# duyhominhnguyen/conan-fgw

Hardware: AMD Instinct MI355X
Metric: molecules/s (K=5 conformers) (higher is better)
Workload: dtype f32

## Files before the change

conan-fgw_amd/csrc/fgw_common.h:

```cpp
#pragma once
#include <type_traits>
#include "common.h"

#ifdef CONAN_FGW_PROFILE
static __device__ long long g_fgw_prof[32];
#define FGW_PROF_ACCESSOR(name)                                                          \
    extern "C" int name(long long *out, int reset) {                                     \
        if (out && hipMemcpyFromSymbol(out, HIP_SYMBOL(g_fgw_prof), sizeof(long long) * 32) != hipSuccess) return -2; \
        if (reset) { long long z[32] = {0}; if (hipMemcpyToSymbol(HIP_SYMBOL(g_fgw_prof), z, sizeof(z)) != hipSuccess) return -2; } \
        return 0;                                                                        \
    }
static __device__ long long g_fgw_trace[2 + 6 * 8192];
#define FGW_PROF_TRACE_ACCESSOR(name)                                                    \
    extern "C" int name(long long *out, int reset) {                                     \
        if (out && hipMemcpyFromSymbol(out, HIP_SYMBOL(g_fgw_trace), sizeof(long long) * (2 + 6 * 8192)) != hipSuccess) return -2; \
        if (reset) { long long z[2] = {0, 0}; if (hipMemcpyToSymbol(HIP_SYMBOL(g_fgw_trace), z, sizeof(z)) != hipSuccess) return -2; } \
        return 0;                                                                        \
    }
#define FGW_PROF_TRACE(tag)                                                              \
    do {                                                                                 \
        if (threadIdx.x == 0) {                                                          \
            const unsigned long long i_ = atomicAdd(reinterpret_cast<unsigned long long *>(&g_fgw_trace[0]), 1ull); \
            if (i_ < 8192) {                                                             \
                long long *r_ = &g_fgw_trace[2 + 6 * i_];                                \
// ... 100 lines not shown
    const double n = rint(t);
    const float f = (float)(t - n);
    const float e = __builtin_amdgcn_exp2f(f);
    return ldexp((double)e, (int)n);
}

__device__ __forceinline__ double exp_fast(double x) {
    const double xc = fmin(fmax(x, -700.0), 700.0);
    const double t = xc * 1.4426950408889634074;
    const double sh = t + 6755399441055744.0;
    const int n = __double2loint(sh);
    const double f = t - (sh - 6755399441055744.0);
    const double e = (double)__builtin_amdgcn_exp2f((float)f);
    const double scale = __hiloint2double((n + 1023) << 20, 0);
    const double r = e * scale;
    return x > -700.0 ? (x < 700.0 ? r : __builtin_inf()) : 0.0;
}

__device__ __forceinline__ double rcp_pos(double s) {
    double r = __builtin_amdgcn_rcp(s);
    r = fma(fma(-s, r, 1.0), r, r);
    r = fma(fma(-s, r, 1.0), r, r);
    return r;
}

__device__ __forceinline__ double log_acc(double s) {
    const double y0 = (double)(__builtin_amdgcn_logf((float)s) * 0.693147180559945309f);
    const double r = s * exp_acc(-y0) - 1.0;
    return y0 + (r - 0.5 * r * r);
}

__device__ __forceinline__ double wave_sum_d(double v) {
#pragma unroll
    for (int o = 32; o > 0; o >>= 1) v += __shfl_xor(v, o, 64);
    return v;
}
__device__ __forceinline__ double wave_max_d(double v) {
#pragma unroll
    for (int o = 32; o > 0; o >>= 1) { double w = __shfl_xor(v, o, 64); v = w > v ? w : v; }
    return v;
}

template <int NW = FGW_WAVES>
__device__ __forceinline__ double block_sum_d(double v, double *red) {
    v = wave_sum_d(v);
    __syncthreads();
    if ((threadIdx.x & 63) == 0) red[threadIdx.x >> 6] = v;
    __syncthreads();
    double s = 0.0;
#pragma unroll
    for (int w = 0; w < NW; ++w) s += red[w];
    return s;
}


typedef double f64x4 __attribute__((ext_vector_type(4)));

__device__ __forceinline__ double exp_lse(double x) {
    const float f = (float)x;
    return (double)__builtin_amdgcn_exp2f(f * 1.44269504088896340736f);
}

template <int NW = FGW_WAVES, class FX, class FW, class FS>
__device__ __forceinline__ void mm_f64_pad(int M, int Nn, int Kd, FX X, FW W, FS st) {
    const int lane = threadIdx.x & 63, wave = __builtin_amdgcn_readfirstlane((int)(threadIdx.x >> 6));
    const int Mq = (M + 15) >> 4, Nq = (Nn + 15) >> 4;
    const int li = lane & 15, lk = lane >> 4;
    for (int t = wave; t < Mq * Nq; t += NW) {
        const int i0 = (t / Nq) << 4, j0 = (t % Nq) << 4;
        const int ia = i0 + li, jb = j0 + li;
        const bool ra = ia < M, cb = jb < Nn;
        const int ic = ra ? ia : M - 1, jc = cb ? jb : Nn - 1;
        f64x4 acc = {0.0, 0.0, 0.0, 0.0};
        int k0 = 0;
        for (; k0 + 16 <= Kd; k0 += 16) {
            double a[4], b[4];
#pragma unroll
            for (int u = 0; u < 4; ++u) { a[u] = X(ic, k0 + 4 * u + lk); b[u] = W(k0 + 4 * u + lk, jc); }
#pragma unroll
            for (int u = 0; u < 4; ++u) acc = __builtin_amdgcn_mfma_f64_16x16x4f64(ra ? a[u] : 0.0, cb ? b[u] : 0.0, acc, 0, 0, 0);
        }
        if (k0 < Kd) {
            double a[4], b[4];
#pragma unroll
            for (int u = 0; u < 4; ++u) {
                const int k = k0 + 4 * u + lk, kc = k < Kd ? k : Kd - 1;
                a[u] = X(ic, kc); b[u] = W(kc, jc);
            }
#pragma unroll
            for (int u = 0; u < 4; ++u) {
                const bool kin = k0 + 4 * u + lk < Kd;
                if (k0 + 4 * u < Kd)
                    acc = __builtin_amdgcn_mfma_f64_16x16x4f64((ra && kin) ? a[u] : 0.0, (cb && kin) ? b[u] : 0.0, acc, 0, 0, 0);
            }
        }
#pragma unroll
        for (int q = 0; q < 4; ++q) {
            const int i = i0 + lk + 4 * q;
            if (i < M && cb) st(i, jb, acc[q]);
        }
    }
}

template <int NW, bool WT, typename TX, typename TW, class FS>
__device__ __forceinline__ void mm_f64_glb(int M, int Nn, int Kd, const TX *__restrict__ X, int pX, const TW *__restrict__ W, int pW, FS st,
                                           const int tid = threadIdx.x) {
    const int lane = tid & 63, wave = __builtin_amdgcn_readfirstlane(tid >> 6);
    const int Mq = (M + 15) >> 4, Nq = (Nn + 15) >> 4;
    const int li = lane & 15, lk = lane >> 4;
    for (int t = wave; t < Mq * Nq; t += NW) {
        const int i0 = (t / Nq) << 4, j0 = (t % Nq) << 4;
        const int ia = i0 + li, jb = j0 + li;
        const bool ra = ia < M, cb = jb < Nn;
        const TX *xr = X + (size_t)(ra ? ia : M - 1) * pX;
        const int jc = cb ? jb : Nn - 1;
        f64x4 acc = {0.0, 0.0, 0.0, 0.0}, acc2 = {0.0, 0.0, 0.0, 0.0};
        for (int k0 = 0; k0 < Kd; k0 += 16) {
            const int kb = k0 + 4 * lk;
            double a[4], b[4];
            if (k0 + 16 <= Kd) {
#pragma unroll
                for (int u = 0; u < 4; ++u) a[u] = (double)xr[kb + u];
                if (WT) {
                    const TW *wr = W + (size_t)jc * pW + kb;
#pragma unroll
                    for (int u = 0; u < 4; ++u) b[u] = (double)wr[u];
                } else {
#pragma unroll
                    for (int u = 0; u < 4; ++u) b[u] = (double)W[(size_t)(kb + u) * pW + jc];
                }
            } else {
#pragma unroll
                for (int u = 0; u < 4; ++u) {
                    const int k = kb + u, kc = k < Kd ? k : Kd - 1;
                    const double av = (double)xr[kc], bv = (double)(WT ? W[(size_t)jc * pW + kc] : W[(size_t)kc * pW + jc]);
                    a[u] = k < Kd ? av : 0.0; b[u] = k < Kd ? bv : 0.0;
                }
            }
            acc = __builtin_amdgcn_mfma_f64_16x16x4f64(ra ? a[0] : 0.0, cb ? b[0] : 0.0, acc, 0, 0, 0);
            acc2 = __builtin_amdgcn_mfma_f64_16x16x4f64(ra ? a[1] : 0.0, cb ? b[1] : 0.0, acc2, 0, 0, 0);
            acc = __builtin_amdgcn_mfma_f64_16x16x4f64(ra ? a[2] : 0.0, cb ? b[2] : 0.0, acc, 0, 0, 0);
            acc2 = __builtin_amdgcn_mfma_f64_16x16x4f64(ra ? a[3] : 0.0, cb ? b[3] : 0.0, acc2, 0, 0, 0);
        }
#pragma unroll
        for (int q = 0; q < 4; ++q) {
            const int i = i0 + lk + 4 * q;
            if (i < M && cb) st(i, jb, acc[q] + acc2[q]);
        }
    }
}

template <int NT>
__device__ __forceinline__ void fgw_order_by_size(const FgwAdj &adj, int B, int K, int tid) {
    static_assert(NT >= 256, "one thread per size bin");
    __shared__ unsigned char nsz[4096];
    __shared__ int hist[256], base[256];
    if (B > 4096) return;
    for (int t = tid; t < 256; t += NT) hist[t] = 0;
    __syncthreads();
    for (int m = tid; m < B; m += NT) {
        const int n = min(max(adj.gptr[m * K + 1] - adj.gptr[m * K], 0), 255);
        nsz[m] = (unsigned char)n;
        atomicAdd(&hist[n], 1);
    }
    __syncthreads();
    if (tid == 0) {
        int run = 0;
        for (int v = 255; v >= 0; --v) { base[v] = run; run += hist[v]; }
    }
    __syncthreads();
    if (tid < 256 && hist[tid] > 0) {
        int pos = base[tid];
        for (int m = 0; m < B; ++m)
            if (nsz[m] == (unsigned char)tid) adj.order[pos++] = m;
    }
}

#ifndef CONAN_FGW_KT
#define CONAN_FGW_KT 2
#endif
template <int NW, bool WT, typename TX, typename TW, class FS, int KT = CONAN_FGW_KT>
__device__ __forceinline__ void mm_f64_glb22(int M, int Nn, int Kd, const TX *__restrict__ X, int pX, const TW *__restrict__ W, int pW, FS st,
                                             const int tid = threadIdx.x) {
    const int lane = tid & 63, wave = __builtin_amdgcn_readfirstlane(tid >> 6);
    const int Mq = (M + 15) >> 4, Nq = (Nn + 15) >> 4;
    const int li = lane & 15, lk = lane >> 4;
    const int Mb = Mq >> 1, Nb = Nq >> 1;
    const int nblk = Mb * Nb, nblk_used = (nblk / NW) * NW;
    auto load_a = [&](const TX *xr, int kb, int k0, double (&a)[KT]) {
        if (k0 + 4 * KT <= Kd) {
#pragma unroll
            for (int u = 0; u < KT; ++u) a[u] = (double)xr[kb + u];
        } else {
#pragma unroll
            for (int u = 0; u < KT; ++u) { const int k = kb + u; const double v = (double)xr[k < Kd ? k : Kd - 1]; a[u] = k < Kd ? v : 0.0; }
        }
    };
    auto load_b = [&](int jc, int kb, int k0, double (&b)[KT]) {
        if (k0 + 4 * KT <= Kd) {
#pragma unroll
            for (int u = 0; u < KT; ++u) b[u] = (double)(WT ? W[(size_t)jc * pW + kb + u] : W[(size_t)(kb + u) * pW + jc]);
        } else {
#pragma unroll
            for (int u = 0; u < KT; ++u) {
                const int k = kb + u, kc = k < Kd ? k : Kd - 1;
                const double v = (double)(WT ? W[(size_t)jc * pW + kc] : W[(size_t)kc * pW + jc]);
                b[u] = k < Kd ? v : 0.0;
            }
        }
    };
    auto store_tile = [&](int i0, int j0, const f64x4 &r) {
        const int jb = j0 + li;
        if (jb < Nn) {
#pragma unroll
            for (int q = 0; q < 4; ++q) { const int i = i0 + lk + 4 * q; if (i < M) st(i, jb, r[q]); }
        }
    };
    for (int t = wave; t < nblk_used; t += NW) {
        const int i0 = (t / Nb) << 5, j0 = (t % Nb) << 5;
        const TX *x0 = X + (size_t)min(i0 + li, M - 1) * pX, *x1 = X + (size_t)min(i0 + 16 + li, M - 1) * pX;
        const int jc0 = min(j0 + li, Nn - 1), jc1 = min(j0 + 16 + li, Nn - 1);
        f64x4 c00 = {0.0, 0.0, 0.0, 0.0}, c01 = c00, c10 = c00, c11 = c00;
        for (int k0 = 0; k0 < Kd; k0 += 4 * KT) {
            const int kb = k0 + KT * lk;
            double a0[KT], a1[KT], b0[KT], b1[KT];
            load_a(x0, kb, k0, a0); load_a(x1, kb, k0, a1); load_b(jc0, kb, k0, b0); load_b(jc1, kb, k0, b1);
#pragma unroll
            for (int u = 0; u < KT; ++u) {
                c00 = __builtin_amdgcn_mfma_f64_16x16x4f64(a0[u], b0[u], c00, 0, 0, 0);
                c01 = __builtin_amdgcn_mfma_f64_16x16x4f64(a0[u], b1[u], c01, 0, 0, 0);
                c10 = __builtin_amdgcn_mfma_f64_16x16x4f64(a1[u], b0[u], c10, 0, 0, 0);
                c11 = __builtin_amdgcn_mfma_f64_16x16x4f64(a1[u], b1[u], c11, 0, 0, 0);
            }
        }
        store_tile(i0, j0, c00); store_tile(i0, j0 + 16, c01); store_tile(i0 + 16, j0, c10); store_tile(i0 + 16, j0 + 16, c11);
    }
    const int rest_blk = nblk - nblk_used;
    const int n_single = rest_blk * 4 + (Mq * Nq - 4 * nblk);
    for (int t = wave; t < n_single; t += NW) {
        int ti, tj;
        if (t < rest_blk * 4) { const int bq = nblk_used + (t >> 2); ti = 2 * (bq / Nb) + ((t >> 1) & 1); tj = 2 * (bq % Nb) + (t & 1); }
        else {
            int q = t - rest_blk * 4;
            const int ncol = (Nq & 1) ? Mq : 0;
            if (q < ncol) { ti = q; tj = Nq - 1; }
            else { q -= ncol; ti = Mq - 1; tj = q; }
        }
        const int i0 = ti << 4, j0 = tj << 4;
        const TX *xr = X + (size_t)min(i0 + li, M - 1) * pX;
        const int jc = min(j0 + li, Nn - 1);
        f64x4 acc = {0.0, 0.0, 0.0, 0.0}, acc2 = {0.0, 0.0, 0.0, 0.0};
        for (int k0 = 0; k0 < Kd; k0 += 4 * KT) {
            const int kb = k0 + KT * lk;
            double a[KT], bq[KT];
            load_a(xr, kb, k0, a); load_b(jc, kb, k0, bq);
#pragma unroll
            for (int u = 0; u < KT; ++u) {
                if (u & 1) acc2 = __builtin_amdgcn_mfma_f64_16x16x4f64(a[u], bq[u], acc2, 0, 0, 0);
                else acc = __builtin_amdgcn_mfma_f64_16x16x4f64(a[u], bq[u], acc, 0, 0, 0);
            }
        }
        store_tile(i0, j0, acc + acc2);
    }
}

typedef int fgw_i32x4 __attribute__((ext_vector_type(4)));
__device__ __forceinline__ void fgw_digit_planes4(const double (&v)[4], double scale, unsigned (&pl)[4]) {
    unsigned r[4];
#pragma unroll
    for (int u = 0; u < 4; ++u) r[u] = ((unsigned)__double2int_rn(v[u] * scale) + 0x00808080u) ^ 0x00808080u;
    const unsigned t0 = __builtin_amdgcn_perm(r[1], r[0], 0x05010400u), t1 = __builtin_amdgcn_perm(r[1], r[0], 0x07030602u);
    const unsigned t2 = __builtin_amdgcn_perm(r[3], r[2], 0x05010400u), t3 = __builtin_amdgcn_perm(r[3], r[2], 0x07030602u);
    pl[0] = __builtin_amdgcn_perm(t2, t0, 0x05040100u); pl[1] = __builtin_amdgcn_perm(t2, t0, 0x07060302u);
    pl[2] = __builtin_amdgcn_perm(t3, t1, 0x05040100u); pl[3] = __builtin_amdgcn_perm(t3, t1, 0x07060302u);
}
template <int NT>
__device__ __forceinline__ void fgw_digits_from_f64(int M, int Kd, const double *__restrict__ X, int pX, int xexp, uint4 *__restrict__ D, const int tid = threadIdx.x) {
    const int KB = ((Kd + 31) >> 5) << 2;
    const double scale = __longlong_as_double((long long)(1023 + 31 - xexp) << 52);
    constexpr int R = 2;
    for (int base = 0; base < M * KB; base += R * NT) {
        double v[R][8];
#pragma unroll
        for (int q = 0; q < R; ++q) {
            const int idx = base + q * NT + tid;
            const int ic = idx < M * KB ? idx : M * KB - 1;
            const int i = ic / KB, kb = ic - i * KB;
            const double *xr = X + (size_t)i * pX;
#pragma unroll
            for (int u = 0; u < 8; ++u) { const int k = 8 * kb + u; v[q][u] = xr[k < Kd ? k : Kd - 1]; }
        }
#pragma unroll
        for (int q = 0; q < R; ++q) {
            const int idx = base + q * NT + tid;
            if (idx >= M * KB) continue;
            const int kb = idx % KB;
            double v0[4], v1[4];
#pragma unroll
            for (int u = 0; u < 4; ++u) { v0[u] = 8 * kb + u < Kd ? v[q][u] : 0.0; v1[u] = 8 * kb + 4 + u < Kd ? v[q][4 + u] : 0.0; }
            unsigned lo[4], hi[4];
            fgw_digit_planes4(v0, scale, lo); fgw_digit_planes4(v1, scale, hi);
            D[2 * idx] = make_uint4(lo[0], hi[0], lo[1], hi[1]);
            D[2 * idx + 1] = make_uint4(lo[2], hi[2], lo[3], hi[3]);
        }
    }
}
__device__ __forceinline__ long fgw_bytes8(const unsigned char *__restrict__ w, int kb, int Kd) {
    unsigned lo = 0, hi = 0;
#pragma unroll
    for (int u = 0; u < 4; ++u) {
        const int k0 = kb + u, k1 = kb + 4 + u;
        lo |= (unsigned)w[k0 < Kd ? k0 : Kd - 1] << (8 * u);
        hi |= (unsigned)w[k1 < Kd ? k1 : Kd - 1] << (8 * u);
    }
    return (long)(((unsigned long long)hi << 32) | lo);
}
template <int NW, class FS>
__device__ __forceinline__ void mm_adj_i8(int M, int Nn, int Kd, const uint4 *__restrict__ D, const unsigned char *__restrict__ Wb, int pW, int xexp, FS st,
                                          const int tid = threadIdx.x) {
    const int lane = tid & 63, wave = __builtin_amdgcn_readfirstlane(tid >> 6);
    const int li = lane & 15, lg = lane >> 4;
    const int Mq = (M + 15) >> 4, Nh = (Nn + 31) >> 5, KB = ((Kd + 31) >> 5) << 2;
    const double unscale = __longlong_as_double((long long)(1023 + xexp - 31) << 52);
    for (int t = wave; t < Mq * Nh; t += NW) {
        const int i0 = (t / Nh) << 4, j0 = (t % Nh) << 5;
        const uint4 *dr = D + (size_t)min(i0 + li, M - 1) * KB * 2;
        const unsigned char *w0 = Wb + (size_t)min(j0 + li, Nn - 1) * pW, *w1 = Wb + (size_t)min(j0 + 16 + li, Nn - 1) * pW;
// ... 559 lines not shown
```

conan-fgw_amd/csrc/fgw_small.hip:

```cpp
#include "fgw_common.h"

#ifdef CONAN_FGW_PROFILE
FGW_PROF_ACCESSOR(conan_debug_fgw_prof)
FGW_PROF_TRACE_ACCESSOR(conan_debug_fgw_trace)
#endif

namespace {

constexpr int SK_SCRATCH_DOUBLES = 3 * 256 + 2 * 64;

template <int R, bool KL, bool SECOND = false>
__global__ void __launch_bounds__(FGW_THREADS, (SECOND || R > 9) ? 1 : 3) k_fgw_coupling_small(
    const float *__restrict__ Ys, const float *__restrict__ Cs, const float *__restrict__ ps, const float *__restrict__ pb,
    FgwDims D, conan_fgw_params prm, int outer, int y_zero, const double *__restrict__ Cw, const double *__restrict__ Yw,
    const int *__restrict__ active, float *__restrict__ Tw, int *__restrict__ info, fgw_part_t *__restrict__ Ypart,
    fgw_part_t *__restrict__ Cpart, const double *__restrict__ zvec, const double *__restrict__ yvec, const int *__restrict__ only, FgwAdj adj) {
    extern __shared__ __attribute__((aligned(16))) char smem[];
    auto solve = [&](const int cid) {
    const int b = cid / D.K, s = cid % D.K;
    if (!fgw_active(active, D.B, b, outer)) return;
    const int N = D.N, P = D.P, d = D.d;
    const int NN = N * N, NP = N * P;
    const int tid = threadIdx.x, lane = tid & 63, w = __builtin_amdgcn_readfirstlane(tid >> 6);
    const bool lane_ok = lane < N;
// ... 663 lines not shown
            if (!have_colp) {
                double pc = 0.0;
                if (ii == 0) {
                    gvP[permL] = lq_ok ? (lq == nbq ? (double)m_pad : 1.0) : 0.0;
                }
                pc = dotR(kA, gw);
                *bufCw = pc;
                __syncthreads();
                colp = ((bufC[lq] + bufC[64 + lq]) + bufC[128 + lq]) + bufC[192 + lq];
            }
            have_colp = false;
            if (__any(lq_ok && !(colp > 1e-150 && colp < 1e150))) { bail = true; break; }
            f = lq_ok ? qj * rcp_pos(colp) : 0.0;
            fvP[permL] = f;
            *bufRw = dotR(kB, fw);
            __syncthreads();
            const double rs = ((bufR[lq] + bufR[64 + lq]) + bufR[128 + lq]) + bufR[192 + lq];
            if (__any(lq_ok && !(rs > 1e-150 && rs < 1e150))) { bail = true; break; }
            g = lq_ok ? pi_l * rcp_pos(rs) : 0.0;
            gvP[permL] = g;
            if (ii % 10 == 0) {
                *bufCw = dotR(kA, gw);
                __syncthreads();
                colp = ((bufC[lq] + bufC[64 + lq]) + bufC[128 + lq]) + bufC[192 + lq];
                have_colp = true;
                double df = lq_ok ? f * colp - qj : 0.0;
                df = df * df;
                if (lq == nbq) df /= (double)m_pad;
                df = wave_sum_d(df);
                if (sqrt(df) < fc.stop_thr) { ++ii; break; }
            }
        }
        if (bail) break;
        sk_total += ii;
        FGW_PROF(6);
        double e2 = 0.0;
        {
            float *trow = Tl + wq * P + lq;
#pragma unroll
            for (int r = 0; r < R; ++r) {
                const bool ok = lq_ok && wq + 4 * r < N;
                float *tp = ok ? trow + 4 * r * P : t_dummy;
                const float tn = (float)((gw[r] * kA[r]) * f);
                double df = ok ? (double)tn - (double)*tp : 0.0;
                df *= df;
                if (nbq >= 0) {
                    const double im = 1.0 / (double)m_pad;
                    df *= (lq == nbq ? im : 1.0) * (wq + 4 * r == nbq ? im : 1.0);
                }
                e2 += df;
                *tp = tn;
            }
        }
        if (cpt % 10 == 0) err = sqrt(block_sum_d(e2, red));
        else __syncthreads();
        ++cpt;
        FGW_PROF(7);
    }
    if (bail) {
        if (tid == 0) { redo[cid] = 1; atomicOr(&info[b * 4 + 3], 1); }
        return;
    }
    __syncthreads();
    {
        int te = tid;
        asm volatile("" : "+v"(te));
        int i = te / N, j = te - i * N;
        const int dq = FGW_THREADS / N, dr = FGW_THREADS - dq * N;
        if (m_pad) {
            const float im = (float)(1.0 / mult);
            for (int t = te; t < NN; t += FGW_THREADS) {
                Tg[t] = Tl[min(i, nb) * P + min(j, nb)] * ((i >= nb ? im : 1.0f) * (j >= nb ? im : 1.0f));
                j += dr; i += dq;
                if (j >= N) { j -= N; ++i; }
            }
        } else {
            for (int t = te; t < NN; t += FGW_THREADS) {
                Tg[t] = Tl[i * P + j];
                j += dr; i += dq;
                if (j >= N) { j -= N; ++i; }
            }
        }
    }
    if (tid == 0) { atomicAdd(&info[b * 4 + 1], cpt); atomicAdd(&info[b * 4 + 2], sk_total); redo[cid] = 0; if (m_pad) atomicOr(&info[b * 4 + 3], 2); }
    FGW_PROF(8);

    if (!prm.fixed_features && Ypart) {
        fgw_part_t *Yp = Ypart + ((size_t)b * D.K + s) * N * d;
        if (yz_lds) {
            const int Nd = N * d;
            for (int t0 = tid; t0 < Nd; t0 += 4 * FGW_THREADS) {
                float zv[4];
#pragma unroll
                for (int u = 0; u < 4; ++u) { const int t = t0 + u * FGW_THREADS; zv[u] = Z[t < Nd ? t : Nd - 1]; }
#pragma unroll
                for (int u = 0; u < 4; ++u) { const int t = t0 + u * FGW_THREADS; if (t < Nd) Zl[t] = zv[u]; }
            }
            __syncthreads();
            mm_lds2<FGW_WAVES, 1, 0, false, false>(N, d, N, Tl, P, Zl, d, [] {}, [&](int i, int c, double v) { Yp[(size_t)i * d + c] = (fgw_part_t)v; });
        } else {
            mm_f64(N, d, N, [&](int i, int k) { return (double)Tl[i * P + k]; }, [&](int k, int c) { return (double)Z[(size_t)k * d + c]; },
                   [&](int i, int c, double v) { Yp[(size_t)i * d + c] = (fgw_part_t)v; });
        }
    }
    FGW_PROF(9);
    if (!prm.fixed_structure) {
        fgw_part_t *Cp = Cpart + ((size_t)b * D.K + s) * NN;
        if (complete) {
            {
                const int lc = lane < Nx ? lane : Nx - 1;
                const float *tr = Tl + lc * P + w;
                double p0 = 0.0, p1 = 0.0;
#pragma unroll
                for (int r = 0; r < R; ++r) {
                    const int q = w + 4 * r;
                    if (q < n_real) { if (r & 1) p1 += (double)tr[4 * r]; else p0 += (double)tr[4 * r]; }
                }
                if (lane < Nx) rsum[w * N + lane] = p0 + p1;
            }
            __syncthreads();
            mm_lds2<FGW_WAVES, 1, 0, true, false>(Nx, Nx, n_real, Tl, P, Tl, P, [] {}, [&](int i, int j, double v) {
                const double ti = ((rsum[i] + rsum[N + i]) + rsum[2 * N + i]) + rsum[3 * N + i];
                const double tj = ((rsum[j] + rsum[N + j]) + rsum[2 * N + j]) + rsum[3 * N + j];
                if (m_pad) Bl[i * P + j] = ti * tj - v;
                else Cp[i * N + j] = (fgw_part_t)(ti * tj - v);
            });
        } else {
            mm_lds2<FGW_WAVES, 1, 0, false, false>(Nx, Nx, Nx, Tl, P, C2l, P, [] {}, [&](int i, int j, double v) { AKl[i * P + j] = v; });
            __syncthreads();
            mm_lds2<FGW_WAVES, 1, 0, true, false>(Nx, Nx, Nx, AKl, P, Tl, P, [] {}, [&](int i, int j, double v) {
                if (m_pad) Bl[i * P + j] = v;
                else Cp[i * N + j] = (fgw_part_t)v;
            });
        }
        if (m_pad) {
            __syncthreads();
            const double im = 1.0 / mult;
            int i = tid / N, j = tid - i * N;
            const int dq = FGW_THREADS / N, dr = FGW_THREADS - dq * N;
            for (int t = tid; t < NN; t += FGW_THREADS) {
                Cp[t] = (fgw_part_t)(Bl[min(i, nb) * P + min(j, nb)] * ((i >= nb ? im : 1.0) * (j >= nb ? im : 1.0)));
                j += dr; i += dq;
                if (j >= N) { j -= N; ++i; }
            }
        }
    }
    FGW_PROF(10);
    FGW_PROF_FLUSH;
    FGW_PROF_TRACE(Nx | (cpt << 8) | (sk_total << 20));
}

template <int NT>
__device__ __forceinline__ void molecule_vectors(const double *__restrict__ Y, const double *__restrict__ C, const float *__restrict__ p, int N,
                                                 int d, bool kl, double *__restrict__ out, int which = 2) {
    constexpr int LPI = NT / 64;
    const int i = (int)threadIdx.x / LPI, sub = (int)threadIdx.x % LPI;
    double y2 = 0.0, r1 = 0.0;
    if (i < N) {
        if (which != 1)
            for (int c = sub; c < d; c += LPI) { const double v = Y[(size_t)i * d + c]; y2 += v * v; }
        if (which != 0)
            for (int k = sub; k < N; k += LPI) {
                const double c1 = C[i * N + k], pk = p ? (double)p[k] : 1.0 / (double)N;
                r1 += (kl ? c1 * log(c1 + 1e-15) - c1 : c1 * c1) * pk;
            }
    }
#pragma unroll
    for (int o = 1; o < LPI; o <<= 1) { y2 += __shfl_xor(y2, o, 64); r1 += __shfl_xor(r1, o, 64); }
    if (i < N && sub == 0) { if (which != 1) out[i] = y2; if (which != 0) out[N + i] = r1; }
}

__global__ void __launch_bounds__(256) k_fgw_small_vectors(const float *__restrict__ Ys, const float *__restrict__ Cs, const float *__restrict__ ps,
                                                           const float *__restrict__ pb, FgwDims D, int kl, double *__restrict__ Cw,
                                                           double *__restrict__ Yw, double *__restrict__ zvec, double *__restrict__ yvec,
                                                           const float *__restrict__ init_C, const float *__restrict__ init_Y, int max_iter,
                                                           int *__restrict__ active, int *__restrict__ info, float *__restrict__ errs,
                                                           float *__restrict__ Yout, float *__restrict__ Cout, FgwAdj adj) {
    const int b = blockIdx.x / D.K, s = blockIdx.x % D.K;
    const int N = D.N, d = D.d;
    __shared__ __attribute__((aligned(16))) unsigned char cm[64 * 65 + 16];
    const int Pm = D.P;
    if (adj.rowptr) {
        for (int t = threadIdx.x; t < (64 * 65 + 16) / 4; t += 256) reinterpret_cast<unsigned *>(cm)[t] = 0u;
        __syncthreads();
        adj_scatter_lds_bytes<256>(adj, (int)blockIdx.x, N, Pm, cm, (int)threadIdx.x);
        __syncthreads();
    }
    if (s == 0) {
        const int NN = N * N, Nd = N * d;
        const float *c0 = init_C ? init_C + (size_t)b * NN : Cs + (size_t)b * D.K * NN;
        for (int t = threadIdx.x; t < NN; t += 256) {
            const float cv = (!init_C && adj.rowptr) ? (float)cm[(t / N) * Pm + (t % N)] : c0[t];
            Cw[(size_t)b * NN + t] = (double)cv; Cout[(size_t)b * NN + t] = cv;
        }
        for (int t = threadIdx.x; t < Nd; t += 256) {
            const float y = init_Y ? init_Y[(size_t)b * Nd + t] : 0.f;
            Yw[(size_t)b * Nd + t] = (double)y; Yout[(size_t)b * Nd + t] = y;
        }
        if (threadIdx.x == 0) { fgw_active_init(active, D.B, b); info[b * 4 + 0] = 0; info[b * 4 + 1] = 0; info[b * 4 + 2] = 0; info[b * 4 + 3] = 0; }
        for (int t = threadIdx.x; t < 2 * max_iter; t += 256) errs[(size_t)b * 2 * max_iter + t] = __builtin_nanf("");
        __syncthreads();
    }
    const float *Z = Ys + ((size_t)b * D.K + s) * N * d;
    const float *C2 = Cs + ((size_t)b * D.K + s) * N * N;
    const float *q = ps ? ps + ((size_t)b * D.K + s) * N : nullptr;
    const int j = (int)threadIdx.x >> 2, sub = (int)threadIdx.x & 3;
    double z2 = 0.0, r2 = 0.0;
    if (j < N) {
        for (int c = sub; c < d; c += 4) { const double v = (double)Z[(size_t)j * d + c]; z2 += v * v; }
        for (int k = sub; k < N; k += 4) {
            const double c2 = adj.rowptr ? (double)cm[j * Pm + k] : (double)C2[j * N + k], qk = q ? (double)q[k] : 1.0 / (double)N;
            r2 += qk * (kl ? c2 : c2 * c2);
        }
    }
    z2 += __shfl_xor(z2, 1, 64); z2 += __shfl_xor(z2, 2, 64);
    r2 += __shfl_xor(r2, 1, 64); r2 += __shfl_xor(r2, 2, 64);
    double *zo = zvec + ((size_t)b * D.K + s) * 2 * N;
    if (j < N && sub == 0) { zo[j] = z2; zo[N + j] = r2; }
    if (s == 0)
        molecule_vectors<256>(Yw + (size_t)b * N * d, Cw + (size_t)b * N * N, pb ? pb + (size_t)b * N : nullptr, N, d, kl != 0, yvec + (size_t)b * 2 * N);
    if (adj.order && blockIdx.x == gridDim.x - 1) fgw_order_by_size<256>(adj, D.B, D.K, (int)threadIdx.x);
}

constexpr int UPD_THREADS = 512;
template <bool Y_FROM_T>
__global__ void __launch_bounds__(UPD_THREADS) k_fgw_update_parts(
    const float *__restrict__ pb, const float *__restrict__ lambdas, FgwDims D, conan_fgw_params prm, int outer,
    const fgw_part_t *__restrict__ Ypart, const fgw_part_t *__restrict__ Cpart, double *__restrict__ Cw, double *__restrict__ Yw,
    int *__restrict__ active, int *__restrict__ info, float *__restrict__ errs, float *__restrict__ Yout, float *__restrict__ Cout,
    double *__restrict__ yvec, const float *__restrict__ Tw, const float *__restrict__ Ys, int chunk) {
    __shared__ double red[UPD_THREADS / 64 + 1];
    extern __shared__ __attribute__((aligned(16))) char usmem[];
    const int part = (int)blockIdx.x >= D.B ? 1 : 0;
    const int b = (int)blockIdx.x - part * D.B;
    const int N = D.N, d = D.d, K = D.K, NN = N * N, Nd = N * d;
    const int tid = threadIdx.x;
    int *flag_out = active + (outer & 1) * 2 * D.B + part * D.B + b;
    if (!fgw_active(active, D.B, b, outer)) {
        if (tid == 0) *flag_out = 0;
        return;
    }
    constexpr int U = 4;
    double e2 = 0.0;
    if (part == 0) {
        if (!prm.fixed_features) {
            double *Yb = Yw + (size_t)b * Nd;
            if constexpr (Y_FROM_T) {
                float *Tl = reinterpret_cast<float *>(usmem), *Zl = Tl + (size_t)chunk * NN;
                const int lane = tid & 63, wave = __builtin_amdgcn_readfirstlane(tid >> 6), li = lane & 15, lk = lane >> 4;
                const int Mq = (N + 15) >> 4, Nq = (d + 15) >> 4;
                constexpr int NWU = UPD_THREADS / 64, TW = 2;
                for (int t0 = 0; t0 < Mq * Nq; t0 += NWU * TW) {
                    int ti0[TW], tj0[TW], tic[TW], tjc[TW];
                    bool mine[TW];
                    f64x4 sum[TW];
#pragma unroll
                    for (int w = 0; w < TW; ++w) {
                        const int t = t0 + wave + w * NWU;
                        mine[w] = t < Mq * Nq;
                        ti0[w] = mine[w] ? (t / Nq) << 4 : 0; tj0[w] = mine[w] ? (t % Nq) << 4 : 0;
                        tic[w] = min(ti0[w] + li, N - 1); tjc[w] = min(tj0[w] + li, d - 1);
                        sum[w] = f64x4{0.0, 0.0, 0.0, 0.0};
                    }
                    for (int s0 = 0; s0 < K; s0 += chunk) {
                        const int cs = min(chunk, K - s0);
                        __syncthreads();
                        const float *tg = Tw + ((size_t)b * K + s0) * NN, *zg = Ys + ((size_t)b * K + s0) * Nd;
                        auto stage = [&](const float *__restrict__ src, float *dst, int n) {
                            constexpr int SB = 12;
                            for (int base = 0; base < n; base += SB * UPD_THREADS) {
                                float v[SB];
#pragma unroll
                                for (int u = 0; u < SB; ++u) { const int q = base + u * UPD_THREADS + tid; v[u] = src[q < n ? q : n - 1]; }
#pragma unroll
                                for (int u = 0; u < SB; ++u) { const int q = base + u * UPD_THREADS + tid; if (q < n) dst[q] = v[u]; }
                            }
                        };
                        stage(tg, Tl, cs * NN);
                        stage(zg, Zl, cs * Nd);
                        __syncthreads();
#pragma unroll
                        for (int w = 0; w < TW; ++w)
                            if (mine[w])
                                for (int q = 0; q < cs; ++q) {
                                    const double lam = lambdas ? (double)lambdas[s0 + q] : 1.0 / (double)K;
                                    const f64x4 r = mm2_tile<0, false>(Tl + (size_t)q * NN + tic[w] * N + lk, Zl + (size_t)q * Nd + lk * d + tjc[w], d, N, lk);
                                    sum[w] = sum[w] + lam * r;
                                }
                    }
#pragma unroll
                    for (int w = 0; w < TW; ++w) {
                        const int jb = tj0[w] + li;
                        if (mine[w] && jb < d) {
#pragma unroll
                            for (int qq = 0; qq < 4; ++qq) {
                                const int i = ti0[w] + lk + 4 * qq;
                                if (i < N) {
                                    const double pw = pb ? (double)pb[(size_t)b * N + i] : 1.0 / (double)N;
                                    const double yn = sum[w][qq] * (pw > 0.0 ? 1.0 / pw : 0.0);
                                    const double df = yn - Yb[i * d + jb];
                                    e2 += df * df;
                                    Yb[i * d + jb] = yn;
                                    Yout[(size_t)b * Nd + i * d + jb] = (float)yn;
                                }
                            }
                        }
                    }
                }
            } else {
                for (int t0 = tid; t0 < Nd; t0 += U * UPD_THREADS) {
                    double acc[U], old[U];
#pragma unroll
                    for (int u = 0; u < U; ++u) {
                        const int t = t0 + u * UPD_THREADS;
                        acc[u] = 0.0; old[u] = 0.0;
                        if (t < Nd) {
                            old[u] = Yb[t];
                            for (int s = 0; s < K; ++s) {
                                const double lam = lambdas ? (double)lambdas[s] : 1.0 / (double)K;
                                const int i = t / d;
                                const double pw = pb ? (double)pb[(size_t)b * N + i] : 1.0 / (double)N;
                                const double pinv = pw > 0.0 ? 1.0 / pw : 0.0;
                                acc[u] += lam * Ypart[((size_t)b * K + s) * Nd + t] * pinv;
                            }
                        }
                    }
#pragma unroll
                    for (int u = 0; u < U; ++u) {
                        const int t = t0 + u * UPD_THREADS;
                        if (t < Nd) {
                            const double df = acc[u] - old[u];
                            e2 += df * df;
                            Yb[t] = acc[u];
                            Yout[(size_t)b * Nd + t] = (float)acc[u];
                        }
                    }
                }
            }
        }
    } else if (!prm.fixed_structure) {
        double *Cb = Cw + (size_t)b * NN;
        for (int t0 = tid; t0 < NN; t0 += U * UPD_THREADS) {
            double acc[U], old[U];
#pragma unroll
            for (int u = 0; u < U; ++u) {
                const int t = t0 + u * UPD_THREADS;
                acc[u] = 0.0; old[u] = 0.0;
                if (t < NN) {
                    old[u] = Cb[t];
                    for (int s = 0; s < K; ++s) {
                        const double lam = lambdas ? (double)lambdas[s] : 1.0 / (double)K;
                        acc[u] += lam * Cpart[((size_t)b * K + s) * NN + t];
                    }
                }
            }
#pragma unroll
            for (int u = 0; u < U; ++u) {
                const int t = t0 + u * UPD_THREADS;
                if (t < NN) {
                    const int i = t / N, j = t - i * N;
                    const double pi = pb ? (double)pb[(size_t)b * N + i] : 1.0 / (double)N;
                    const double pj = pb ? (double)pb[(size_t)b * N + j] : 1.0 / (double)N;
                    const double cn = pi * pj > 0.0 ? (prm.loss_fun ? exp(acc[u] / (pi * pj)) : acc[u] / (pi * pj)) : 0.0;
                    const double df = cn - old[u];
                    e2 += df * df;
                    Cb[t] = cn;
                    Cout[(size_t)b * NN + t] = (float)cn;
                }
            }
        }
    }
    const double err = sqrt(block_sum_d<UPD_THREADS / 64>(e2, red));
    if (yvec) molecule_vectors<UPD_THREADS>(Yw + (size_t)b * Nd, Cw + (size_t)b * NN, pb ? pb + (size_t)b * N : nullptr, N, d, prm.loss_fun != 0,
                                            yvec + (size_t)b * 2 * N, part);
    if (tid == 0) {
        errs[((size_t)b * 2 + part) * prm.max_iter + outer] = (float)err;
        info[b * 4 + 0] = outer + 1;
        *flag_out = err > (double)prm.tol ? 1 : 0;
    }
}

inline size_t small_lds(int N, int d) {
    const size_t NP = (size_t)N * fgw_pitch(N);
    (void)d; return NP * 8 * 4 + (256 + 128 + 8 + (NP >= (size_t)SK_SCRATCH_DOUBLES ? 0 : SK_SCRATCH_DOUBLES)) * 8 + NP * 4 * 2;
}

}

bool conan_fgw_small_supported(int N, int d) { return N <= 64 && small_lds(N, d) <= 160 * 1024; }

void conan_fgw_small_prepare(const FgwCall &c) {
    k_fgw_small_vectors<<<c.D.B * c.D.K, 256, 0, c.s>>>(c.Ys, c.Cs, c.ps, c.p, c.D, c.prm.loss_fun, c.Cw, c.Yw, c.zvec, c.yvec, c.init_C, c.init_Y,
                                                       c.prm.max_iter, c.active, c.info, c.errs, c.Y, c.C, c.adj);
}

template <class F>
static void with_rows(int R, F &&f) {
    if (R <= 6) f(std::integral_constant<int, 6>{});
    else if (R <= 9) f(std::integral_constant<int, 9>{});
    else if (R <= 12) f(std::integral_constant<int, 12>{});
    else f(std::integral_constant<int, 16>{});
}

template <int R, typename C2T>
static void launch_fast(const FgwCall &c, int outer, int y_zero, fgw_part_t *Ypart) {
    const FgwDims &D = c.D;
    const int tpw = fast_tiles_per_wave(D.N);
    auto go = [&](auto kernel) {
        launch_lds(kernel, D.B * D.K, FGW_THREADS, fast_lds<C2T>(D.N).bytes, c.s, c.Ys, c.Cs, c.ps, c.p, D, c.prm, fast_const(c.prm, D.N), outer,
                   y_zero, c.Cw, c.Yw, c.active, c.T, c.info, Ypart, c.Cpart, c.zvec, c.yvec, c.redo, c.adj);
    };
    if constexpr (R <= 6) go(k_fgw_coupling_fast<R, 1, C2T>);
    else if constexpr (R <= 12) { if (tpw <= 1) go(k_fgw_coupling_fast<R, 1, C2T>); else go(k_fgw_coupling_fast<R, 3, C2T>); }
    else { if (tpw <= 1) go(k_fgw_coupling_fast<R, 1, C2T>); else if (tpw <= 3) go(k_fgw_coupling_fast<R, 3, C2T>); else go(k_fgw_coupling_fast<R, 4, C2T>); }
}

bool conan_fgw_fast_supported(int N, int d, int small_int) {
    if (N > 64 || N < 4) return false;
    const size_t lds = small_int ? fast_lds<unsigned char>(N).bytes : fast_lds<float>(N).bytes;
    return lds <= 160 * 1024 && d >= 1;
}

void conan_fgw_small_coupling(const FgwCall &c, int outer, int y_zero, fgw_part_t *Ypart) {
    const FgwDims &D = c.D;
    const size_t lds = small_lds(D.N, D.d);
    const int grid = D.B * D.K;
    const bool kl = c.prm.loss_fun != 0;
    with_rows((D.N + 3) / 4, [&](auto R) {
        const int *only = nullptr;
        if (!kl && conan_fgw_fast_supported(D.N, D.d, c.prm.cs_small_int)) {
            if (c.prm.cs_small_int) launch_fast<R.value, unsigned char>(c, outer, y_zero, Ypart);
            else launch_fast<R.value, float>(c, outer, y_zero, Ypart);
            only = c.redo;
        }
        auto exact = [&](auto kernel, int blocks) {
            launch_lds(kernel, blocks, FGW_THREADS, lds, c.s, c.Ys, c.Cs, c.ps, c.p, D, c.prm, outer, y_zero, c.Cw, c.Yw, c.active, c.T, c.info, Ypart,
                       c.Cpart, c.zvec, c.yvec, only, c.adj);
        };
        if (kl) exact(k_fgw_coupling_small<R.value, true, false>, grid);
        else if (only) exact(k_fgw_coupling_small<R.value, false, true>, (grid + 63) / 64);
        else exact(k_fgw_coupling_small<R.value, false, false>, grid);
    });
}

void conan_fgw_small_update(const FgwCall &c, int outer, bool y_from_t) {
    const FgwDims &D = c.D;
    const int chunk = y_from_t ? conan_fgw_update_chunk(D.K, D.N, D.d, D.B) : 0;
    if (chunk > 0)
        launch_lds(k_fgw_update_parts<true>, 2 * D.B, UPD_THREADS, (size_t)chunk * ((size_t)D.N * D.N + (size_t)D.N * D.d) * 4, c.s, c.p, c.lambdas, D,
                   c.prm, outer, nullptr, c.Cpart, c.Cw, c.Yw, c.active, c.info, c.errs, c.Y, c.C, c.yvec, c.T, c.Ys, chunk);
    else
        k_fgw_update_parts<false><<<2 * D.B, UPD_THREADS, 0, c.s>>>(c.p, c.lambdas, D, c.prm, outer, c.Ypart, c.Cpart, c.Cw, c.Yw, c.active, c.info, c.errs,
                                                                     c.Y, c.C, c.yvec, nullptr, nullptr, 0);
}

int conan_fgw_update_chunk(int K, int N, int d, int B) {
    if (N > 64) return 0;
    const size_t per = ((size_t)N * N + (size_t)N * d) * 4, budget = (2 * B <= 256 ? 144 : 72) * 1024;
    if (per > budget) return 0;
    const int c = (int)(budget / per);
    return c < K ? c : K;
}
```

Measured before the change: 118,200.

## Parallelize size ordering, fuse T/Z staging and reuse LDS results in update

Replaces the serial per-bin scan in fgw_order_by_size with a parallel prefix scan and a wavefront-level packed-byte rank, and runs it in a dedicated extra workgroup at the start of the grid instead of the last block. The update kernel now stages T and Z in one fused batched loop, issues its global loads before checking the active flag, and prefetches the old Y values and pb entries. It also writes the updated Y and C into LDS so molecule_vectors reads them from there rather than from global memory, and adds an occupancy hint to the launch bounds. The intent is to cut serial latency and global round trips, at the cost of extra LDS, more registers and loads issued for inactive molecules.

```diff
diff --git a/conan-fgw_amd/csrc/fgw_common.h b/conan-fgw_amd/csrc/fgw_common.h
--- a/conan-fgw_amd/csrc/fgw_common.h
+++ b/conan-fgw_amd/csrc/fgw_common.h
@@ -276,27 +276,72 @@
 
 template <int NT>
 __device__ __forceinline__ void fgw_order_by_size(const FgwAdj &adj, int B, int K, int tid) {
-    static_assert(NT >= 256, "one thread per size bin");
-    __shared__ unsigned char nsz[4096];
-    __shared__ int hist[256], base[256];
+    static_assert(NT >= 256 && NT % 64 == 0 && 4096 % NT == 0, "one thread per size bin, whole wavefronts, whole rounds");
+    constexpr int NWV = NT / 64, RB = 4;
+    __shared__ __attribute__((aligned(4))) unsigned char nsz[4096];
+    __shared__ int hist[256], next[256], scan[2][256];
+    __shared__ unsigned wcnt[NWV * 64];
     if (B > 4096) return;
     for (int t = tid; t < 256; t += NT) hist[t] = 0;
     __syncthreads();
-    for (int m = tid; m < B; m += NT) {
-        const int n = min(max(adj.gptr[m * K + 1] - adj.gptr[m * K], 0), 255);
-        nsz[m] = (unsigned char)n;
-        atomicAdd(&hist[n], 1);
+    for (int m0 = 0; m0 < B; m0 += RB * NT) {
+        int lo[RB], hi[RB];
+#pragma unroll
+        for (int r = 0; r < RB; ++r) {
+            const int m = min(m0 + r * NT + tid, B - 1);
+            lo[r] = adj.gptr[m * K]; hi[r] = adj.gptr[m * K + 1];
+        }
+#pragma unroll
+        for (int r = 0; r < RB; ++r) {
+            const int m = m0 + r * NT + tid;
+            if (m < B) {
+                const int n = min(max(hi[r] - lo[r], 0), 255);
+                nsz[m] = (unsigned char)n;
+                atomicAdd(&hist[n], 1);
+            }
+        }
     }
     __syncthreads();
-    if (tid == 0) {
-        int run = 0;
-        for (int v = 255; v >= 0; --v) { base[v] = run; run += hist[v]; }
-    }
+    if (tid < 256) scan[0][tid] = hist[255 - tid];
     __syncthreads();
-    if (tid < 256 && hist[tid] > 0) {
-        int pos = base[tid];
-        for (int m = 0; m < B; ++m)
-            if (nsz[m] == (unsigned char)tid) adj.order[pos++] = m;
+    int src = 0;
+    for (int off = 1; off < 256; off <<= 1) {
+        if (tid < 256) scan[src ^ 1][tid] = scan[src][tid] + (tid >= off ? scan[src][tid - off] : 0);
+        __syncthreads();
+        src ^= 1;
+    }
+    if (tid < 256) next[255 - tid] = scan[src][tid] - hist[255 - tid];
+    const int lane = tid & 63, wv = tid >> 6;
+    for (int m0 = 0; m0 < B; m0 += NT) {
+        for (int t = tid; t < NWV * 64; t += NT) wcnt[t] = 0u;
+        __syncthreads();
+        const int m = m0 + tid;
+        const bool on = m < B;
+        const int n = on ? (int)nsz[m] : 0;
+        if (on) atomicAdd(&wcnt[wv * 64 + (n >> 2)], 1u << (8 * (n & 3)));
+        int before = 0;
+        const unsigned *row = reinterpret_cast<const unsigned *>(nsz) + ((m0 + wv * 64) >> 2);
+        const unsigned n4 = (unsigned)n * 0x01010101u;
+#pragma unroll
+        for (int q = 0; q < 16; ++q) {
+            const unsigned x = row[q] ^ n4;
+            const unsigned eq = ~((((x & 0x7f7f7f7fu) + 0x7f7f7f7fu) | x) | 0x7f7f7f7fu);
+            const int k = min(max(lane - 4 * q, 0), 4);
+            before += __popc(eq & (unsigned)(0x80808080ull & ((1ull << (8 * k)) - 1ull)));
+        }
+        __syncthreads();
+        if (on) {
+            int pos = next[n] + before;
+            for (int w = 0; w < wv; ++w) pos += (int)((wcnt[w * 64 + (n >> 2)] >> (8 * (n & 3))) & 255u);
+            adj.order[pos] = m;
+        }
+        int add = 0;
+        if (tid < 256) {
+#pragma unroll
+            for (int w = 0; w < NWV; ++w) add += (int)((wcnt[w * 64 + (tid >> 2)] >> (8 * (tid & 3))) & 255u);
+        }
+        __syncthreads();
+        if (tid < 256) next[tid] += add;
     }
 }
 
diff --git a/conan-fgw_amd/csrc/fgw_small.hip b/conan-fgw_amd/csrc/fgw_small.hip
--- a/conan-fgw_amd/csrc/fgw_small.hip
+++ b/conan-fgw_amd/csrc/fgw_small.hip
@@ -839,16 +839,17 @@
 
 template <int NT>
 __device__ __forceinline__ void molecule_vectors(const double *__restrict__ Y, const double *__restrict__ C, const float *__restrict__ p, int N,
-                                                 int d, bool kl, double *__restrict__ out, int which = 2) {
+                                                 int d, bool kl, double *__restrict__ out, int which,
+                                                 int pY, int pC) {
     constexpr int LPI = NT / 64;
     const int i = (int)threadIdx.x / LPI, sub = (int)threadIdx.x % LPI;
     double y2 = 0.0, r1 = 0.0;
     if (i < N) {
         if (which != 1)
-            for (int c = sub; c < d; c += LPI) { const double v = Y[(size_t)i * d + c]; y2 += v * v; }
+            for (int c = sub; c < d; c += LPI) { const double v = Y[(size_t)i * pY + c]; y2 += v * v; }
         if (which != 0)
             for (int k = sub; k < N; k += LPI) {
-                const double c1 = C[i * N + k], pk = p ? (double)p[k] : 1.0 / (double)N;
+                const double c1 = C[i * pC + k], pk = p ? (double)p[k] : 1.0 / (double)N;
                 r1 += (kl ? c1 * log(c1 + 1e-15) - c1 : c1 * c1) * pk;
             }
     }
@@ -863,14 +864,16 @@
                                                            const float *__restrict__ init_C, const float *__restrict__ init_Y, int max_iter,
                                                            int *__restrict__ active, int *__restrict__ info, float *__restrict__ errs,
                                                            float *__restrict__ Yout, float *__restrict__ Cout, FgwAdj adj) {
-    const int b = blockIdx.x / D.K, s = blockIdx.x % D.K;
+    const int wg = (int)blockIdx.x - (adj.order ? 1 : 0);
+    if (wg < 0) { fgw_order_by_size<256>(adj, D.B, D.K, (int)threadIdx.x); return; }
+    const int b = wg / D.K, s = wg % D.K;
     const int N = D.N, d = D.d;
     __shared__ __attribute__((aligned(16))) unsigned char cm[64 * 65 + 16];
     const int Pm = D.P;
     if (adj.rowptr) {
         for (int t = threadIdx.x; t < (64 * 65 + 16) / 4; t += 256) reinterpret_cast<unsigned *>(cm)[t] = 0u;
         __syncthreads();
-        adj_scatter_lds_bytes<256>(adj, (int)blockIdx.x, N, Pm, cm, (int)threadIdx.x);
+        adj_scatter_lds_bytes<256>(adj, wg, N, Pm, cm, (int)threadIdx.x);
         __syncthreads();
     }
     if (s == 0) {
@@ -905,17 +908,16 @@
     double *zo = zvec + ((size_t)b * D.K + s) * 2 * N;
     if (j < N && sub == 0) { zo[j] = z2; zo[N + j] = r2; }
     if (s == 0)
-        molecule_vectors<256>(Yw + (size_t)b * N * d, Cw + (size_t)b * N * N, pb ? pb + (size_t)b * N : nullptr, N, d, kl != 0, yvec + (size_t)b * 2 * N);
-    if (adj.order && blockIdx.x == gridDim.x - 1) fgw_order_by_size<256>(adj, D.B, D.K, (int)threadIdx.x);
+        molecule_vectors<256>(Yw + (size_t)b * N * d, Cw + (size_t)b * N * N, pb ? pb + (size_t)b * N : nullptr, N, d, kl != 0, yvec + (size_t)b * 2 * N, 2, d, N);
 }
 
 constexpr int UPD_THREADS = 512;
 template <bool Y_FROM_T>
-__global__ void __launch_bounds__(UPD_THREADS) k_fgw_update_parts(
+__global__ void __launch_bounds__(UPD_THREADS, 4) k_fgw_update_parts(
     const float *__restrict__ pb, const float *__restrict__ lambdas, FgwDims D, conan_fgw_params prm, int outer,
     const fgw_part_t *__restrict__ Ypart, const fgw_part_t *__restrict__ Cpart, double *__restrict__ Cw, double *__restrict__ Yw,
     int *__restrict__ active, int *__restrict__ info, float *__restrict__ errs, float *__restrict__ Yout, float *__restrict__ Cout,
-    double *__restrict__ yvec, const float *__restrict__ Tw, const float *__restrict__ Ys, int chunk) {
+    double *__restrict__ yvec, const float *__restrict__ Tw, const float *__restrict__ Ys, int chunk, int y_lds) {
     __shared__ double red[UPD_THREADS / 64 + 1];
     extern __shared__ __attribute__((aligned(16))) char usmem[];
     const int part = (int)blockIdx.x >= D.B ? 1 : 0;
@@ -923,10 +925,14 @@
     const int N = D.N, d = D.d, K = D.K, NN = N * N, Nd = N * d;
     const int tid = threadIdx.x;
     int *flag_out = active + (outer & 1) * 2 * D.B + part * D.B + b;
-    if (!fgw_active(active, D.B, b, outer)) {
+    const bool act = fgw_active(active, D.B, b, outer);
+    const bool late = Y_FROM_T && (part == 0 ? !prm.fixed_features : !prm.fixed_structure);
+    if (!late && !act) {
         if (tid == 0) *flag_out = 0;
         return;
     }
+    double *const Xl = reinterpret_cast<double *>(usmem);
+    const int dP = d | 1, nP = N | 1;
     constexpr int U = 4;
     double e2 = 0.0;
     if (part == 0) {
@@ -949,23 +955,42 @@
                         tic[w] = min(ti0[w] + li, N - 1); tjc[w] = min(tj0[w] + li, d - 1);
                         sum[w] = f64x4{0.0, 0.0, 0.0, 0.0};
                     }
+                    double yold[TW][4];
                     for (int s0 = 0; s0 < K; s0 += chunk) {
                         const int cs = min(chunk, K - s0);
+                        if (t0 | s0) __syncthreads();
+                        const float *tg = Tw + ((size_t)b * K + s0) * NN, *zg = Ys + ((size_t)b * K + s0) * Nd;
+                        {
+                            constexpr int ST = 11, SZ = 21;
+                            const int nT = cs * NN, nZ = cs * Nd;
+                            for (int bt = 0, bz = 0; bt < nT || bz < nZ; bt += ST * UPD_THREADS, bz += SZ * UPD_THREADS) {
+                                float vt[ST], vz[SZ];
+#pragma unroll
+                                for (int u = 0; u < ST; ++u) vt[u] = tg[min(bt + u * UPD_THREADS + tid, nT - 1)];
+#pragma unroll
+                                for (int u = 0; u < SZ; ++u) vz[u] = zg[min(bz + u * UPD_THREADS + tid, nZ - 1)];
+                                if (late && !(t0 | s0 | bt) && !act) {
+                                    if (tid == 0) *flag_out = 0;
+                                    return;
+                                }
+#pragma unroll
+                                for (int u = 0; u < ST; ++u) { const int q = bt + u * UPD_THREADS + tid; if (q < nT) Tl[q] = vt[u]; }
+#pragma unroll
+                                for (int u = 0; u < SZ; ++u) { const int q = bz + u * UPD_THREADS + tid; if (q < nZ) Zl[q] = vz[u]; }
+                            }
+                        }
                         __syncthreads();
-                        const float *tg = Tw + ((size_t)b * K + s0) * NN, *zg = Ys + ((size_t)b * K + s0) * Nd;
-                        auto stage = [&](const float *__restrict__ src, float *dst, int n) {
-                            constexpr int SB = 12;
-                            for (int base = 0; base < n; base += SB * UPD_THREADS) {
-                                float v[SB];
-#pragma unroll
-                                for (int u = 0; u < SB; ++u) { const int q = base + u * UPD_THREADS + tid; v[u] = src[q < n ? q : n - 1]; }
-#pragma unroll
-                                for (int u = 0; u < SB; ++u) { const int q = base + u * UPD_THREADS + tid; if (q < n) dst[q] = v[u]; }
-                            }
-                        };
-                        stage(tg, Tl, cs * NN);
-                        stage(zg, Zl, cs * Nd);
-                        __syncthreads();
+                        if (s0 + chunk >= K) {
+                            int lkq = lk;
+                            asm volatile("" : "+v"(lkq));
+#pragma unroll
+                            for (int w = 0; w < TW; ++w)
+#pragma unroll
+                                for (int qq = 0; qq < 4; ++qq) {
+                                    const int ic = min(ti0[w] + lkq + 4 * qq, N - 1);
+                                    yold[w][qq] = Yb[ic * d + tjc[w]];
+                                }
+                        }
 #pragma unroll
                         for (int w = 0; w < TW; ++w)
                             if (mine[w])
@@ -975,6 +1000,10 @@
                                     sum[w] = sum[w] + lam * r;
                                 }
                     }
+                    if (y_lds) __syncthreads();
+                    int Nu = N;
+                    asm volatile("" : "+s"(Nu));
+                    const double pw_uniform = 1.0 / (double)Nu;
 #pragma unroll
                     for (int w = 0; w < TW; ++w) {
                         const int jb = tj0[w] + li;
@@ -983,12 +1012,13 @@
                             for (int qq = 0; qq < 4; ++qq) {
                                 const int i = ti0[w] + lk + 4 * qq;
                                 if (i < N) {
-                                    const double pw = pb ? (double)pb[(size_t)b * N + i] : 1.0 / (double)N;
+                                    const double pw = pb ? (double)pb[(size_t)b * N + i] : pw_uniform;
                                     const double yn = sum[w][qq] * (pw > 0.0 ? 1.0 / pw : 0.0);
-                                    const double df = yn - Yb[i * d + jb];
+                                    const double df = yn - yold[w][qq];
                                     e2 += df * df;
                                     Yb[i * d + jb] = yn;
                                     Yout[(size_t)b * Nd + i * d + jb] = (float)yn;
+                                    if (y_lds) Xl[i * dP + jb] = yn;
                                 }
                             }
                         }
@@ -1027,39 +1057,52 @@
         }
     } else if (!prm.fixed_structure) {
         double *Cb = Cw + (size_t)b * NN;
-        for (int t0 = tid; t0 < NN; t0 += U * UPD_THREADS) {
+        for (int r0 = 0; r0 < NN; r0 += U * UPD_THREADS) {
+            const int t0 = r0 + tid;
             double acc[U], old[U];
+            float pfi[U], pfj[U];
 #pragma unroll
             for (int u = 0; u < U; ++u) {
                 const int t = t0 + u * UPD_THREADS;
-                acc[u] = 0.0; old[u] = 0.0;
+                acc[u] = 0.0; old[u] = 0.0; pfi[u] = 0.f; pfj[u] = 0.f;
                 if (t < NN) {
                     old[u] = Cb[t];
+                    if (pb) { const int i = t / N; pfi[u] = pb[(size_t)b * N + i]; pfj[u] = pb[(size_t)b * N + (t - i * N)]; }
                     for (int s = 0; s < K; ++s) {
                         const double lam = lambdas ? (double)lambdas[s] : 1.0 / (double)K;
                         acc[u] += lam * Cpart[((size_t)b * K + s) * NN + t];
                     }
                 }
             }
+            if (late && r0 == 0 && !act) {
+                if (tid == 0) *flag_out = 0;
+                return;
+            }
 #pragma unroll
             for (int u = 0; u < U; ++u) {
                 const int t = t0 + u * UPD_THREADS;
                 if (t < NN) {
                     const int i = t / N, j = t - i * N;
-                    const double pi = pb ? (double)pb[(size_t)b * N + i] : 1.0 / (double)N;
-                    const double pj = pb ? (double)pb[(size_t)b * N + j] : 1.0 / (double)N;
+                    const double pi = pb ? (double)pfi[u] : 1.0 / (double)N;
+                    const double pj = pb ? (double)pfj[u] : 1.0 / (double)N;
                     const double cn = pi * pj > 0.0 ? (prm.loss_fun ? exp(acc[u] / (pi * pj)) : acc[u] / (pi * pj)) : 0.0;
                     const double df = cn - old[u];
                     e2 += df * df;
                     Cb[t] = cn;
                     Cout[(size_t)b * NN + t] = (float)cn;
+                    if (Y_FROM_T) Xl[i * nP + j] = cn;
                 }
             }
         }
     }
     const double err = sqrt(block_sum_d<UPD_THREADS / 64>(e2, red));
-    if (yvec) molecule_vectors<UPD_THREADS>(Yw + (size_t)b * Nd, Cw + (size_t)b * NN, pb ? pb + (size_t)b * N : nullptr, N, d, prm.loss_fun != 0,
-                                            yvec + (size_t)b * 2 * N, part);
+    if (yvec) {
+        const float *pm = pb ? pb + (size_t)b * N : nullptr;
+        double *out = yvec + (size_t)b * 2 * N;
+        if (late && part == 0 && y_lds) molecule_vectors<UPD_THREADS>(Xl, Xl, pm, N, d, prm.loss_fun != 0, out, 0, dP, nP);
+        else if (late && part == 1) molecule_vectors<UPD_THREADS>(Xl, Xl, pm, N, d, prm.loss_fun != 0, out, 1, dP, nP);
+        else molecule_vectors<UPD_THREADS>(Yw + (size_t)b * Nd, Cw + (size_t)b * NN, pm, N, d, prm.loss_fun != 0, out, part, d, N);
+    }
     if (tid == 0) {
         errs[((size_t)b * 2 + part) * prm.max_iter + outer] = (float)err;
         info[b * 4 + 0] = outer + 1;
@@ -1077,7 +1120,7 @@
 bool conan_fgw_small_supported(int N, int d) { return N <= 64 && small_lds(N, d) <= 160 * 1024; }
 
 void conan_fgw_small_prepare(const FgwCall &c) {
-    k_fgw_small_vectors<<<c.D.B * c.D.K, 256, 0, c.s>>>(c.Ys, c.Cs, c.ps, c.p, c.D, c.prm.loss_fun, c.Cw, c.Yw, c.zvec, c.yvec, c.init_C, c.init_Y,
+    k_fgw_small_vectors<<<c.D.B * c.D.K + (c.adj.order ? 1 : 0), 256, 0, c.s>>>(c.Ys, c.Cs, c.ps, c.p, c.D, c.prm.loss_fun, c.Cw, c.Yw, c.zvec, c.yvec, c.init_C, c.init_Y,
                                                        c.prm.max_iter, c.active, c.info, c.errs, c.Y, c.C, c.adj);
 }
 
@@ -1133,12 +1176,16 @@
 void conan_fgw_small_update(const FgwCall &c, int outer, bool y_from_t) {
     const FgwDims &D = c.D;
     const int chunk = y_from_t ? conan_fgw_update_chunk(D.K, D.N, D.d, D.B) : 0;
-    if (chunk > 0)
-        launch_lds(k_fgw_update_parts<true>, 2 * D.B, UPD_THREADS, (size_t)chunk * ((size_t)D.N * D.N + (size_t)D.N * D.d) * 4, c.s, c.p, c.lambdas, D,
-                   c.prm, outer, nullptr, c.Cpart, c.Cw, c.Yw, c.active, c.info, c.errs, c.Y, c.C, c.yvec, c.T, c.Ys, chunk);
-    else
+    if (chunk > 0) {
+        const size_t stage = (size_t)chunk * ((size_t)D.N * D.N + (size_t)D.N * D.d) * 4, budget = (size_t)(2 * D.B <= 256 ? 144 : 72) * 1024;
+        const size_t c_bytes = (size_t)D.N * (D.N | 1) * 8, y_bytes = (size_t)D.N * (D.d | 1) * 8;
+        const int y_lds = y_bytes <= budget && ((D.N + 15) / 16) * ((D.d + 15) / 16) <= 16 ? 1 : 0;
+        const size_t lds = std::max(stage, std::max(c_bytes, y_lds ? y_bytes : (size_t)0));
+        launch_lds(k_fgw_update_parts<true>, 2 * D.B, UPD_THREADS, lds, c.s, c.p, c.lambdas, D,
+                   c.prm, outer, nullptr, c.Cpart, c.Cw, c.Yw, c.active, c.info, c.errs, c.Y, c.C, c.yvec, c.T, c.Ys, chunk, y_lds);
+    } else
         k_fgw_update_parts<false><<<2 * D.B, UPD_THREADS, 0, c.s>>>(c.p, c.lambdas, D, c.prm, outer, c.Ypart, c.Cpart, c.Cw, c.Yw, c.active, c.info, c.errs,
-                                                                     c.Y, c.C, c.yvec, nullptr, nullptr, 0);
+                                                                     c.Y, c.C, c.yvec, nullptr, nullptr, 0, 0);
 }
 
 int conan_fgw_update_chunk(int K, int N, int d, int B) {
```

After: 119,000, median of 6. Within noise of the previous version (+0.7%).
